# ChengeLi/LongTerm360FoV

Hardware: AMD Instinct MI355X
Metric: sequences/sec (batch=1024, T_in=30->T_out=30, h=256) (higher is better)
Workload: dtype f32; 1 GPU; configs[1]: target-only seq2seq inference (encoder + autoregressive decoder), H=256, batch=1024 per GPU, T_in=30->T_out=30, F_enc=90, F_dec=6, fp32, act=sigmoid, impl=auto; global_batch=1024, parallelism=replicas x1 (no collective)

## Files before the change

longterm360fov_amd/csrc/lstm_cluster.hip:

```cpp
#include <stdlib.h>

#include <atomic>
#include <mutex>

#include "fov_common.h"
#include "xch_common.h"

namespace fov {

constexpr int BT = 16;
constexpr int XR = 6;
constexpr int KPAD = 2;
constexpr int NXBUF = 3;
constexpr int CL_MAX_F = 96;
constexpr int CL_MAX_O = 8;
constexpr unsigned SPIN_LIMIT = 1u << 20;

constexpr int MODE_LAYER = 0;
constexpr int MODE_DECODE = 1;
constexpr int MODE_LAYER_ZX = 2;

typedef unsigned u32x2 __attribute__((ext_vector_type(2)));
typedef unsigned u32x4g __attribute__((ext_vector_type(4)));
typedef float f32x2 __attribute__((ext_vector_type(2)));
// ... 25 lines not shown
        if (stamp_on && t < STAMP_STEPS) {                                                      \
            unsigned long long t_;                                                              \
            asm volatile("s_memtime %0\n\ts_waitcnt lgkmcnt(0)" : "=s"(t_)::"memory");          \
            g_stamps[MODE & 1][t][slot] = t_;                                                       \
        }                                                                                       \
        __builtin_amdgcn_sched_barrier(0);                                                      \
    } while (0)
#define FOV_PSTAMP(slot)                                                                        \
    do {                                                                                        \
        __builtin_amdgcn_sched_barrier(0);                                                      \
        if (blockIdx.x == 5 && threadIdx.x == 0) g_stamps[MODE & 1][STAMP_STEPS - 1][slot] = __builtin_amdgcn_s_memtime(); \
        __builtin_amdgcn_sched_barrier(0);                                                      \
    } while (0)
#else
#define FOV_STAMP(slot) do { } while (0)
#define FOV_PSTAMP(slot) do { } while (0)
#endif

struct ClusterLds {
    int ldx, ldh;
    int off_k, off_h, off_x, off_w, off_bd, off_flag, total_floats;
};
__host__ __device__ inline ClusterLds cluster_lds(int H, int F, bool decode) {
    ClusterLds L;
    const int fp = round16(F);
    L.ldx = fp + 4;
    L.ldh = H + 4;
    L.off_k = 0;
    L.off_h = L.off_k + fp * 256 + 4 * KPAD * 256;
    L.off_x = L.off_h + BT * L.ldh;
    L.off_w = L.off_x + NXBUF * BT * L.ldx;
    L.off_bd = L.off_w + (decode ? 2 * 4 * 128 : 0);
    L.off_flag = L.off_bd + 8;
    L.total_floats = L.off_flag + 8 + 64;
    return L;
}

constexpr int MF_MID = 0, MF_FIRST = 1, MF_LAST = 2;
#define FOV_MFMA_STR(pre, post) pre "v_mfma_f32_16x16x4_f32 %0, %1, %2, %0" post
template <bool W_AGPR>
__device__ __forceinline__ void mfma_f32(f32x4& acc, float a, float w, int pos) {
    if constexpr (W_AGPR) {
        if (pos == MF_MID) asm volatile(FOV_MFMA_STR("", "") : "+v"(acc) : "v"(a), "a"(w));
        else if (pos == MF_FIRST) asm volatile(FOV_MFMA_STR("s_nop 1\n\t", "") : "+v"(acc) : "v"(a), "a"(w));
        else if (pos == MF_LAST) asm volatile(FOV_MFMA_STR("", "\n\ts_nop 7\n\ts_nop 3") : "+v"(acc) : "v"(a), "a"(w));
        else asm volatile(FOV_MFMA_STR("s_nop 1\n\t", "\n\ts_nop 7\n\ts_nop 3") : "+v"(acc) : "v"(a), "a"(w));
    } else {
        if (pos == MF_MID) asm volatile(FOV_MFMA_STR("", "") : "+v"(acc) : "v"(a), "v"(w));
        else if (pos == MF_FIRST) asm volatile(FOV_MFMA_STR("s_nop 1\n\t", "") : "+v"(acc) : "v"(a), "v"(w));
        else if (pos == MF_LAST) asm volatile(FOV_MFMA_STR("", "\n\ts_nop 7\n\ts_nop 3") : "+v"(acc) : "v"(a), "v"(w));
        else asm volatile(FOV_MFMA_STR("s_nop 1\n\t", "\n\ts_nop 7\n\ts_nop 3") : "+v"(acc) : "v"(a), "v"(w));
    }
}
__host__ __device__ constexpr int mf_pos(bool first_run, bool last_run, bool is_first, bool is_last) {
    return ((first_run && is_first) ? MF_FIRST : 0) | ((last_run && is_last) ? MF_LAST : 0);
}

template <int H, bool DEC_KMAP, int J0, int J1, bool REST>
__device__ __forceinline__ void load_weights(float (&wR)[H / 16][4][4], float (&bias)[4], float* sKw,
                                             const float* K, const float* R, const float* b, int F, int Fp,
                                             int col0, int slice, int lane) {
    constexpr int G = H / 64;
    const int n = lane & 15, g4 = lane >> 4;
    const int H4 = 4 * H;
    {
        const __amdgpu_buffer_rsrc_t rrs = __builtin_amdgcn_make_buffer_rsrc(const_cast<float*>(R), 0, H * H4 * 4, 0x00020000);
        const unsigned voff = (unsigned)((4 * g4 * H4 + col0 + n) * 4);
#pragma unroll
        for (int j = J0; j < J1; ++j) {
            const unsigned kb = (unsigned)((((slice + (j >> 2)) & (G - 1)) * 64 + (j & 3) * 16) * H4 * 4);
#pragma unroll
            for (int s = 0; s < 4; ++s)
#pragma unroll
                for (int g = 0; g < 4; ++g)
                    wR[j][s][g] = __uint_as_float(__builtin_amdgcn_raw_buffer_load_b32(rrs, voff, kb + (unsigned)((s * H4 + g * H) * 4), 0));
        }
    }
    if constexpr (!REST) return;
    {
        const __amdgpu_buffer_rsrc_t brs = __builtin_amdgcn_make_buffer_rsrc(const_cast<float*>(b), 0, b ? H4 * 4 : 0, 0x00020000);
#pragma unroll
        for (int g = 0; g < 4; ++g) bias[g] = __uint_as_float(__builtin_amdgcn_raw_buffer_load_b32(brs, (unsigned)((g * H + col0 + n) * 4), 0, 0));
    }
    const int nq = Fp >> 4;
    constexpr int QMAX = CL_MAX_F / 16;
    const __amdgpu_buffer_rsrc_t krs = __builtin_amdgcn_make_buffer_rsrc(const_cast<float*>(K), 0, F * H4 * 4, 0x00020000);
    f32x4 kv[DEC_KMAP ? 1 : QMAX][4];
#pragma unroll
    for (int q = 0; q < (DEC_KMAP ? 1 : QMAX); ++q)
#pragma unroll
        for (int s = 0; s < 4; ++s) {
            const int k = DEC_KMAP ? (s < 2 ? 4 * s + g4 : F) : 16 * q + 4 * g4 + s;
            const unsigned voff = (unsigned)((k * H4 + col0 + n) * 4);
#pragma unroll
            for (int g = 0; g < 4; ++g)
                kv[q][s][g] = __uint_as_float(__builtin_amdgcn_raw_buffer_load_b32(krs, voff + (unsigned)(g * H * 4), 0, 0));
        }
#pragma unroll
    for (int q = 0; q < (DEC_KMAP ? 1 : QMAX); ++q)
        if (q < nq) {
#pragma unroll
            for (int s = 0; s < 4; ++s) *(f32x4*)(sKw + ((q * 4 + s) * 64 + lane) * 4) = kv[q][s];
        }
}

template <int H>
__device__ __forceinline__ void load_r_block(float (&wR)[H / 16][4][4], int j, const float* R, int col0, int slice, int lane) {
    constexpr int G = H / 64;
    const int n = lane & 15, g4 = lane >> 4;
    const int H4 = 4 * H;
    const __amdgpu_buffer_rsrc_t rrs = __builtin_amdgcn_make_buffer_rsrc(const_cast<float*>(R), 0, H * H4 * 4, 0x00020000);
    const unsigned voff = (unsigned)((4 * g4 * H4 + col0 + n) * 4);
    const unsigned kb = (unsigned)((((slice + (j >> 2)) & (G - 1)) * 64 + (j & 3) * 16) * H4 * 4);
#pragma unroll
    for (int s = 0; s < 4; ++s)
#pragma unroll
        for (int g = 0; g < 4; ++g)
            wR[j][s][g] = __uint_as_float(__builtin_amdgcn_raw_buffer_load_b32(rrs, voff, kb + (unsigned)((s * H4 + g * H) * 4), 0));
}
template <int H>
__device__ __forceinline__ void load_dec_small(float (&bias)[4], f32x4 (&kb)[2], const float* K, const float* b, int F, int col0, int lane) {
    const int n = lane & 15, g4 = lane >> 4;
    const int H4 = 4 * H;
    const __amdgpu_buffer_rsrc_t brs = __builtin_amdgcn_make_buffer_rsrc(const_cast<float*>(b), 0, b ? H4 * 4 : 0, 0x00020000);
#pragma unroll
    for (int g = 0; g < 4; ++g) bias[g] = __uint_as_float(__builtin_amdgcn_raw_buffer_load_b32(brs, (unsigned)((g * H + col0 + n) * 4), 0, 0));
    const __amdgpu_buffer_rsrc_t krs = __builtin_amdgcn_make_buffer_rsrc(const_cast<float*>(K), 0, F * H4 * 4, 0x00020000);
#pragma unroll
    for (int s = 0; s < 2; ++s) {
        const unsigned voff = (unsigned)(((4 * s + g4) * H4 + col0 + n) * 4);
#pragma unroll
        for (int g = 0; g < 4; ++g) kb[s][g] = __uint_as_float(__builtin_amdgcn_raw_buffer_load_b32(krs, voff + (unsigned)(g * H * 4), 0, 0));
    }
}

template <bool FIRST, bool LAST>
__device__ __forceinline__ void input_proj(f32x4 (&acc)[4], const float* arow, const float* sKw, int nq, int lane) {
    if (nq <= 0) return;
    const float* bl = sKw + lane * 4;
    f32x4 a = *(const f32x4*)arow;
    f32x4 b0 = *(const f32x4*)bl;
    f32x4 b1 = *(const f32x4*)(bl + 256);
    if (FIRST) asm volatile("s_nop 1" : "+v"(acc[0]), "+v"(acc[1]), "+v"(acc[2]), "+v"(acc[3]));
    for (int q = 0; q < nq - 1; ++q) {
        const f32x4 an = *(const f32x4*)(arow + 16 * (q + 1));
        const float* bq = bl + q * 1024;
#pragma unroll
        for (int s = 0; s < 4; ++s) {
            const f32x4 bn = *(const f32x4*)(bq + (s + 2) * 256);
#pragma unroll
            for (int g = 0; g < 4; ++g) mfma_f32<false>(acc[g], a[s], b0[g], MF_MID);
            b0 = b1;
            b1 = bn;
        }
        a = an;
    }
    const float* bq = bl + (nq - 1) * 1024;
#pragma unroll
    for (int s = 0; s < 4; ++s) {
        const f32x4 bn = *(const f32x4*)(bq + (s + 2) * 256);
#pragma unroll
        for (int g = 0; g < 4; ++g) mfma_f32<false>(acc[g], a[s], b0[g], mf_pos(false, LAST, false, s == 3 && g == 3));
        b0 = b1;
        b1 = bn;
    }
}

template <int NQC, bool FIRST, bool LAST>
__device__ __forceinline__ void input_proj_fixed(f32x4 (&acc)[4], const float* arow, const float* sKw, int lane) {
    const float* bl = sKw + lane * 4;
    f32x4 a = *(const f32x4*)arow;
    f32x4 b0 = *(const f32x4*)bl;
    f32x4 b1 = *(const f32x4*)(bl + 256);
#pragma unroll
    for (int q = 0; q < NQC; ++q) {
        f32x4 an = a;
        if (q + 1 < NQC) an = *(const f32x4*)(arow + 16 * (q + 1));
#pragma unroll
        for (int s = 0; s < 4; ++s) {
            f32x4 bn = b1;
            if (4 * q + s + 2 < 4 * NQC) bn = *(const f32x4*)(bl + (4 * q + s + 2) * 256);
#pragma unroll
            for (int g = 0; g < 4; ++g)
                mfma_f32<false>(acc[g], a[s], b0[g], mf_pos(FIRST, LAST, q == 0 && s == 0, q == NQC - 1 && s == 3 && g == 3));
            b0 = b1;
            b1 = bn;
        }
        a = an;
    }
}
template <bool FIRST, bool LAST>
__device__ __forceinline__ void input_proj_any(f32x4 (&acc)[4], const float* arow, const float* sKw, int nq, int lane) {
    if (nq == 6) input_proj_fixed<6, FIRST, LAST>(acc, arow, sKw, lane);
    else input_proj<FIRST, LAST>(acc, arow, sKw, nq, lane);
}

template <bool LAST>
__device__ __forceinline__ void input_proj_reg(f32x4 (&acc)[4], f32x4 y4, const f32x4 (&kb)[2]) {
#pragma unroll
    for (int s = 0; s < 2; ++s)
#pragma unroll
        for (int g = 0; g < 4; ++g) mfma_f32<false>(acc[g], y4[s], kb[s][g], mf_pos(true, LAST, s == 0, s == 1 && g == 3));
}

template <int H, int J0, int J1, bool FIRST, bool LAST>
__device__ __forceinline__ void recurrent(f32x4 (&acc)[4], const float* hrow, const float (&wR)[H / 16][4][4]) {
    if (J0 >= J1) return;
    f32x4 a = *(const f32x4*)(hrow + 16 * J0);
#pragma unroll
    for (int j = J0; j < J1; ++j) {
        f32x4 an = a;
        if (j + 1 < J1) an = *(const f32x4*)(hrow + 16 * (j + 1));
#pragma unroll
        for (int s = 0; s < 4; ++s)
#pragma unroll
            for (int g = 0; g < 4; ++g)
                mfma_f32<true>(acc[g], a[s], wR[j][s][g], mf_pos(FIRST, LAST, j == J0 && s == 0, j == J1 - 1 && s == 3 && g == 3));
        a = an;
    }
}

struct ClusterCarry {
    unsigned epoch;
    XchTicket ticket;
    bool same_xcd, aborted, xch_used;
    float c[4], h[4];
};

template <int H, int ACT, int MODE, int FUSED>
__device__ __forceinline__ void cluster_body(const LstmParams& p, ClusterCarry& cy) {
    constexpr int G = H / 64;
    constexpr int NQ = H / 16;
    constexpr int NG = (G - 1) * 2;
    constexpr bool LAYER = (MODE != MODE_DECODE);
    constexpr bool ZX = (MODE == MODE_LAYER_ZX);
    constexpr bool F1 = (FUSED == 1), F2 = (FUSED == 2);
    extern __shared__ __attribute__((aligned(16))) float smem[];

    const int tid = threadIdx.x, lane = tid & 63, wave = tid >> 6;
    const int n = lane & 15, g4 = lane >> 4;
    constexpr unsigned OORB = 0x80000000u;
#ifdef FOV_STAMPS
    if (blockIdx.x == 5 && tid == 0) g_stamps[MODE & 1][STAMP_STEPS - 1][0] = __builtin_amdgcn_s_memtime();
#endif
    float hcarry[BT * H / 256];
    if constexpr (F2) {
        const ClusterLds L1 = cluster_lds(H, p.F, false);
#pragma unroll
        for (int q = 0; q < BT * H / 256; ++q) {
            const int i = tid + 256 * q;
            hcarry[q] = smem[L1.off_h + (i / H) * L1.ldh + (i - (i / H) * H)];
        }
        __syncthreads();
    }
    int group, slice;
    if (G > 1 && ((p.num_groups & 7) == 0 || p.xcd_pad)) {
        group = (blockIdx.x / (8 * G)) * 8 + (blockIdx.x & 7);
        slice = (blockIdx.x >> 3) & (G - 1);
    } else {
        group = blockIdx.x / G;
        slice = blockIdx.x - group * G;
    }
    const int col0 = slice * 64 + wave * 16;

    const float* Kp = LAYER ? p.K : p.dK;
    const float* Rp = LAYER ? p.R : p.dR;
    const float* bp = LAYER ? p.b : p.db;
    const int F = LAYER ? (ZX ? 0 : p.F) : p.F_dec;
    const int steps = LAYER ? p.T : p.T_out;
    const int Fp = round16(F);
    const int nq = Fp >> 4;

    const ClusterLds L = cluster_lds(H, F, !LAYER);
    const int LDX = L.ldx, LDH = L.ldh;
    float* sK = smem + L.off_k;
    float* sH = smem + L.off_h;
    float* sX = smem + L.off_x;
    float* sY = smem + L.off_w;
    int* sFlag = (int*)(smem + L.off_flag);
    float* sKw = sK + wave * (nq * 4 + KPAD) * 256;

    const bool xch_used = (G > 1) && (!LAYER || p.T > 1 || F1);
    unsigned* sXch = (unsigned*)(sFlag + 4);
    const bool hdr = xch_used && !F2;
    unsigned hdr_base = 0, hdr_launch = 0;
    if (hdr && tid == 0) {
        hdr_base = xch_status_load(p.status + ST_EPOCH);
        hdr_launch = xch_status_load(p.status + ST_LAUNCHES);
    }
    float wR[NQ][4][4];
    float bias[4];
    constexpr int JA = NQ < 3 ? NQ : 3;
    constexpr int STREAM_LA = 3;
    f32x4 kb[2];
    if constexpr (F2) {
        load_dec_small<H>(bias, kb, Kp, bp, F, col0, lane);
    } else {
        load_weights<H, !LAYER, 0, JA, false>(wR, bias, sKw, Kp, Rp, bp, F, Fp, col0, slice, lane);
    }
    unsigned long long* hello = p.xch + (size_t)p.num_groups * 2 * BT * H + (size_t)group * G;
    const unsigned my_xcc = xcc_id();
    if (hdr && tid == 0) {
        sXch[0] = hdr_base;
        sXch[1] = hdr_launch;
        st_granule(hello + slice, (((unsigned long long)hdr_base + 1ull) << 32) | my_xcc);
        xch_count_arrival(p.status);
    }
    FOV_PSTAMP(3);
    if constexpr (!F2) load_weights<H, !LAYER, JA, NQ, true>(wR, bias, sKw, Kp, Rp, bp, F, Fp, col0, slice, lane);
    FOV_PSTAMP(2);
    const bool poisoned = hdr && xch_poisoned(p.status);
    const unsigned arrival = 0;
    if (tid == 0) { sFlag[0] = (poisoned || (F2 && cy.aborted)) ? 1 : 0; sFlag[1] = 0; }
    if (hdr && !poisoned && tid < G) {
        const unsigned long long hello_tag = (unsigned long long)sXch[0] + 1ull;
        unsigned long long hv = 0;
        unsigned spins = 0;
        while (true) {
            hv = ld_granule(hello + tid);
            if ((hv >> 32) == hello_tag) break;
            if (++spins > SPIN_LIMIT || ((spins & 63u) == 0 && xch_poisoned(p.status))) {
                xch_give_up(p.status);
                sFlag[0] = 1;
                break;
            }
            __builtin_amdgcn_s_sleep(4);
        }
        if ((unsigned)hv != my_xcc) sFlag[1] = 1;
    }
    FOV_PSTAMP(4);
    float xpre[2][XR];
    {
        const int xrw0 = tid >> 4, xcl0 = tid & 15;
        const bool xuse0 = LAYER && !ZX;
        const int b00 = group * BT;
        const int live0 = (group < p.num_tiles) ? (p.B - b00 < BT ? p.B - b00 : BT) : 0;
        const __amdgpu_buffer_rsrc_t xg0 = __builtin_amdgcn_make_buffer_rsrc(
            const_cast<float*>(xuse0 && live0 > 0 ? p.x + (size_t)b00 * p.T * F : nullptr), 0, xuse0 ? live0 * p.T * F * 4 : 0, 0x00020000);
#pragma unroll
        for (int tt = 0; tt < 2; ++tt)
#pragma unroll
            for (int i = 0; i < XR; ++i)
                xpre[tt][i] = __uint_as_float(__builtin_amdgcn_raw_buffer_load_b32(
                    xg0, (tt < steps && xcl0 + 16 * i < F) ? (unsigned)((xrw0 * p.T * F + xcl0 + 16 * i) * 4) : OORB, (unsigned)(tt * F * 4), 0));
    }
    for (int i = tid; i < NXBUF * BT * LDX; i += 256) sX[i] = 0.f;

    float wd[4];
    float bd4[4];
    if (!LAYER) {
        const int O = p.F_dec;
        const __amdgpu_buffer_rsrc_t wdrs = __builtin_amdgcn_make_buffer_rsrc(const_cast<float*>(p.dW), 0, H * O * 4, 0x00020000);
        const __amdgpu_buffer_rsrc_t bdrs = __builtin_amdgcn_make_buffer_rsrc(const_cast<float*>(p.dbias), 0, O * 4, 0x00020000);
#pragma unroll
        for (int ss = 0; ss < 4; ++ss) {
            const int unit = col0 + 4 * g4 + ss;
            const int o = 4 * (n & 3) + (n >> 2);
            wd[ss] = __uint_as_float(__builtin_amdgcn_raw_buffer_load_b32(wdrs, (o < O) ? (unsigned)((unit * O + o) * 4) : OORB, 0, 0));
        }
#pragma unroll
        for (int ss = 0; ss < 4; ++ss)
            bd4[ss] = __uint_as_float(__builtin_amdgcn_raw_buffer_load_b32(bdrs, (4 * ss + g4 < O) ? (unsigned)((4 * ss + g4) * 4) : OORB, 0, 0));
    }
    if constexpr (F2) {
#pragma unroll
        for (int j = 0; j < STREAM_LA; ++j) load_r_block<H>(wR, j, Rp, col0, slice, lane);
    } else if (!LAYER) {
        __syncthreads();
        kb[0] = *(const f32x4*)(sKw + lane * 4);
        kb[1] = *(const f32x4*)(sKw + 256 + lane * 4);
    }

    __syncthreads();
    FOV_PSTAMP(5);
    XchTicket ticket = {0u, 0u, 0u};
    if (xch_used && !F2) ticket = xch_ticket(sXch, arrival);
    if constexpr (F2) ticket = cy.ticket;
    unsigned epoch = F2 ? cy.epoch : ticket.base;
    const bool same_xcd = F2 ? cy.same_xcd : (xch_used && (sFlag[1] == 0) && (p.force_safe_exchange == 0));
    bool aborted = F2 ? cy.aborted : (xch_used && sFlag[0] != 0);
    if (xch_used && !F2 && tid == 0 && !same_xcd && !aborted)
        xch_count_safe(p.status, ticket);
#ifdef FOV_STAMPS
    const bool stamp_on = (blockIdx.x == 5 && tid == 0);
#endif
    const float* hrow = sH + n * LDH + 4 * g4;

    const __amdgpu_buffer_rsrc_t xrs = __builtin_amdgcn_make_buffer_rsrc(
        p.xch + (size_t)group * 2 * BT * H, 0, 2 * BT * H * (int)sizeof(unsigned long long), 0x00020000);
    const unsigned pub_off = (unsigned)((2 * g4) * H + col0 + n) * 16u;
    unsigned goff[NG > 0 ? NG : 1];
    int loff[NG > 0 ? NG : 1];
#pragma unroll
    for (int j = 0; j < NG; ++j) {
        const int idx = j * 256 + tid;
        const int rot = (idx >> 9) + 1, within = idx & 511;
        const int osl = (slice + rot) & (G - 1);
        goff[j] = (unsigned)((within >> 6) * H + osl * 64 + (within & 63)) * 16u;
        loff[j] = 2 * (within >> 6) * LDH + rot * 64 + (within & 63);
    }

    constexpr int NYG = (LAYER || G == 1) ? 0 : G;
    const __amdgpu_buffer_rsrc_t yrs = __builtin_amdgcn_make_buffer_rsrc(
        p.xch + (size_t)p.num_groups * 2 * BT * H + (size_t)p.num_groups * G + (size_t)group * 2 * G * 128, 0,
        LAYER ? 0 : 2 * G * 128 * (int)sizeof(unsigned long long), 0x00020000);
    const unsigned ypub_off = (unsigned)((slice * 64 + lane) * 16);
    const unsigned ygoff = (unsigned)(lane * 16);
    constexpr unsigned YPAR_BYTES = G * 64 * 16;
    constexpr int YPAR_LDS = 4 * 128;
    auto own_partial = [&](int par) -> f32x2 {
        const float* yb = sY + par * YPAR_LDS + lane * 2;
        const f32x2 a0 = *(const f32x2*)yb, a1 = *(const f32x2*)(yb + 128), a2 = *(const f32x2*)(yb + 256), a3 = *(const f32x2*)(yb + 384);
        return (a0 + a1) + (a2 + a3);
    };

    const bool h_zero = !F2 && p.h0 == nullptr;
    for (int tile = group; tile < p.num_tiles && !aborted; tile += p.num_groups) {
        const int b0 = tile * BT;
        const int live_rows = p.B - b0 < BT ? p.B - b0 : BT;
        const __amdgpu_buffer_rsrc_t c0rs = __builtin_amdgcn_make_buffer_rsrc(
            const_cast<float*>(p.c0 ? p.c0 + (size_t)b0 * H : nullptr), 0, p.c0 ? live_rows * H * 4 : 0, 0x00020000);
        const __amdgpu_buffer_rsrc_t h0rs = __builtin_amdgcn_make_buffer_rsrc(
            const_cast<float*>(p.h0 ? p.h0 + (size_t)b0 * H : nullptr), 0, p.h0 ? live_rows * H * 4 : 0, 0x00020000);
        float c[4], hcur[4];
#pragma unroll
        for (int r = 0; r < 4; ++r) {
            const unsigned off = (unsigned)(((4 * g4 + r) * H + col0 + n) * 4);
            if constexpr (F2) {
                c[r] = cy.c[r];
                hcur[r] = cy.h[r];
            } else {
                c[r] = __uint_as_float(__builtin_amdgcn_raw_buffer_load_b32(c0rs, off, 0, 0));
                hcur[r] = __uint_as_float(__builtin_amdgcn_raw_buffer_load_b32(h0rs, off, 0, 0));
            }
        }
        {
            float hv[BT * H / 256];
#pragma unroll
            for (int q = 0; q < BT * H / 256; ++q) {
                const int i = tid + 256 * q;
                const int row = i / H, pos = i - row * H;
                const int unit = ((slice + (pos >> 6)) & (G - 1)) * 64 + (pos & 63);
                if constexpr (F2) hv[q] = hcarry[q];
                else hv[q] = h_zero ? 0.f : __uint_as_float(__builtin_amdgcn_raw_buffer_load_b32(h0rs, (unsigned)((row * H + unit) * 4), 0, 0));
            }
#pragma unroll
            for (int q = 0; q < BT * H / 256; ++q) {
                const int i = tid + 256 * q;
                const int row = i / H, pos = i - row * H;
                sH[row * LDH + pos] = hv[q];
            }
        }
        const int xrw = tid >> 4, xcl = tid & 15;
        const bool xuse = LAYER && !ZX;
        const __amdgpu_buffer_rsrc_t xgrs = __builtin_amdgcn_make_buffer_rsrc(
            const_cast<float*>(xuse ? p.x + (size_t)b0 * p.T * F : nullptr), 0, xuse ? live_rows * p.T * F * 4 : 0, 0x00020000);
        unsigned xoff[XR];
#pragma unroll
        for (int i = 0; i < XR; ++i) xoff[i] = (xcl + 16 * i < F) ? (unsigned)((xrw * p.T * F + xcl + 16 * i) * 4) : OORB;
        const __amdgpu_buffer_rsrc_t zxrs = __builtin_amdgcn_make_buffer_rsrc(
            const_cast<float*>(ZX ? p.zx + (size_t)b0 * p.T * 4 * H : nullptr), 0, ZX ? live_rows * p.T * 4 * H * 4 : 0, 0x00020000);
        const unsigned zxoff = (unsigned)((4 * g4 * p.T * 4 * H + col0 + n) * 4);
        f32x4 zr[4];
        float* xl = sX + xrw * LDX + xcl;
        if (xuse) {
            float x2[2][XR];
            if (tile == group) {
#pragma unroll
                for (int tt = 0; tt < 2; ++tt)
#pragma unroll
                    for (int i = 0; i < XR; ++i) x2[tt][i] = xpre[tt][i];
            } else {
#pragma unroll
                for (int tt = 0; tt < 2; ++tt)
#pragma unroll
                    for (int i = 0; i < XR; ++i)
                        x2[tt][i] = __uint_as_float(__builtin_amdgcn_raw_buffer_load_b32(xgrs, tt < steps ? xoff[i] : OORB, (unsigned)(tt * F * 4), 0));
            }
#pragma unroll
            for (int tt = 0; tt < 2; ++tt)
                if (tt < steps) {
#pragma unroll
                    for (int i = 0; i < XR; ++i)
                        if (xcl + 16 * i < F) xl[tt * BT * LDX + 16 * i] = x2[tt][i];
                }
        }
        const __amdgpu_buffer_rsrc_t yors = __builtin_amdgcn_make_buffer_rsrc(
            (!LAYER && p.out) ? p.out + (size_t)b0 * p.T_out * p.F_dec : nullptr, 0, (!LAYER && p.out) ? live_rows * p.T_out * p.F_dec * 4 : 0, 0x00020000);
        unsigned yoff[2];
#pragma unroll
        for (int ss = 0; ss < 2; ++ss)
            yoff[ss] = (!LAYER && 4 * ss + g4 < p.F_dec) ? (unsigned)((n * p.T_out * p.F_dec + 4 * ss + g4) * 4) : OORB;
        f32x4 y4 = (f32x4){0.f, 0.f, 0.f, 0.f};
        if (!LAYER) {
            const __amdgpu_buffer_rsrc_t y0rs = __builtin_amdgcn_make_buffer_rsrc(
                const_cast<float*>(p.dec_in0 + (size_t)b0 * F), 0, live_rows * F * 4, 0x00020000);
#pragma unroll
            for (int ss = 0; ss < 4; ++ss)
                y4[ss] = __uint_as_float(__builtin_amdgcn_raw_buffer_load_b32(y0rs, (4 * ss + g4 < F) ? (unsigned)((n * F + 4 * ss + g4) * 4) : OORB, 0, 0));
        }
        __syncthreads();
        FOV_PSTAMP(6);

        f32x4 acc[4];
#pragma unroll
        for (int g = 0; g < 4; ++g) acc[g] = (f32x4){bias[g], bias[g], bias[g], bias[g]};
        if (ZX && steps > 0) {
#pragma unroll
            for (int g = 0; g < 4; ++g)
#pragma unroll
                for (int r = 0; r < 4; ++r)
                    acc[g][r] = bias[g] + __uint_as_float(__builtin_amdgcn_raw_buffer_load_b32(zxrs, zxoff + (unsigned)((r * p.T * 4 * H + g * H) * 4), 0, 0));
        }
        if (steps > 0) {
            if (LAYER) input_proj_any<true, true>(acc, sX + n * LDX + 4 * g4, sKw, nq, lane);
            else input_proj_reg<true>(acc, y4, kb);
            if constexpr (F2) {
                f32x4 a = *(const f32x4*)hrow;
#pragma unroll
                for (int j = 0; j < NQ; ++j) {
                    if (j + STREAM_LA < NQ) load_r_block<H>(wR, j + STREAM_LA, Rp, col0, slice, lane);
                    f32x4 an = a;
                    if (j + 1 < NQ) an = *(const f32x4*)(hrow + 16 * (j + 1));
#pragma unroll
                    for (int s2 = 0; s2 < 4; ++s2)
#pragma unroll
                        for (int g = 0; g < 4; ++g)
                            mfma_f32<true>(acc[g], a[s2], wR[j][s2][g], mf_pos(false, true, false, j == NQ - 1 && s2 == 3 && g == 3));
                    a = an;
                }
            } else if (!h_zero) {
                recurrent<H, 0, 4, true, true>(acc, hrow, wR);
            }
        }

        float xr[XR];
#pragma unroll
        for (int i = 0; i < XR; ++i) xr[i] = 0.f;
        for (int t = 0; t < steps; ++t) {
            FOV_STAMP(0);
#ifdef FOV_STAMPS
            if (stamp_on && t < STAMP_STEPS) g_stamps[MODE & 1][t][9] = __builtin_amdgcn_s_memrealtime();
#endif
            if (LAYER && !ZX && t > 0 && t + 1 < steps) {
                float* xb = xl + ((t + 1) % 3) * BT * LDX;
#pragma unroll
                for (int i = 0; i < XR; ++i)
                    if (xcl + 16 * i < F) xb[16 * i] = xr[i];
            }
            if (ZX && t + 1 < steps) {
#pragma unroll
                for (int g = 0; g < 4; ++g)
#pragma unroll
                    for (int r = 0; r < 4; ++r)
                        zr[g][r] = bias[g] + __uint_as_float(__builtin_amdgcn_raw_buffer_load_b32(
                                                 zxrs, zxoff + (unsigned)(((r * p.T + (t + 1)) * 4 * H + g * H) * 4), 0, 0));
            }
            if (LAYER && !ZX && t + 2 < steps) {
#pragma unroll
                for (int i = 0; i < XR; ++i)
                    xr[i] = __uint_as_float(__builtin_amdgcn_raw_buffer_load_b32(xgrs, xoff[i], (unsigned)((t + 2) * F * 4), 0));
            }
            if (LAYER || t == 0) {
                if (!((h_zero || F2) && t == 0)) recurrent<H, 4, NQ, true, true>(acc, hrow, wR);
            } else {
                constexpr int JM = 4 + (NQ - 4) / 2;
                recurrent<H, 4, JM, true, false>(acc, hrow, wR);
                u32x4g vy[NYG > 0 ? NYG : 1];
                const unsigned yso = (epoch & 1u) * YPAR_BYTES;
#pragma unroll
                for (int q = 0; q < NYG; ++q) vy[q] = __builtin_amdgcn_raw_buffer_load_b128(yrs, ygoff, yso + (unsigned)(q * 1024), 16);
                recurrent<H, JM, NQ, false, false>(acc, hrow, wR);
                __builtin_amdgcn_sched_barrier(0);
                f32x2 ysum;
                if constexpr (NYG > 0) {
                    unsigned spins = 0;
                    while (true) {
                        bool ok = true;
#pragma unroll
                        for (int q = 0; q < NYG; ++q) ok = ok && (vy[q].y == epoch) && (vy[q].w == epoch);
                        if (__all(ok)) break;
                        if (++spins > SPIN_LIMIT || ((spins & 63u) == 0 && xch_poisoned(p.status))) {
                            if (lane == 0) { xch_give_up(p.status); sFlag[0] = 1; }
// ... 32 lines not shown
                const float ig = acc[0][r], fg = acc[1][r], gg = acc[2][r], og = acc[3][r];
                c[r] = fmaf(fg, c[r], ig * gg);
                hcur[r] = og * c[r];
#else
                const float ig = rec_act<ACT>(acc[0][r]);
                const float fg = rec_act<ACT>(acc[1][r]);
                const float gg = tanh_f(acc[2][r]);
                const float og = rec_act<ACT>(acc[3][r]);
                c[r] = fmaf(fg, c[r], ig * gg);
                hcur[r] = og * tanh_f(c[r]);
#endif
                if (LAYER && p.reserve) {
                    const int row = b0 + 4 * g4 + r;
                    if (row < p.B) {
                        float* rp = p.reserve + (((size_t)row * p.T + t) * 5) * H + col0 + n;
                        rp[0] = ig; rp[H] = fg; rp[2 * H] = gg; rp[3 * H] = og; rp[4 * H] = c[r];
                    }
                }
            }
            unsigned xsoff = 0;
            const bool do_xch = (G > 1) && (!LAYER || t + 1 < steps || F1);
            if (do_xch) {
                ++epoch;
                xsoff = (epoch & 1u) * (unsigned)(BT * H * sizeof(unsigned long long));
                if (same_xcd) {
#pragma unroll
                    for (int r = 0; r < 2; ++r)
                        __builtin_amdgcn_raw_buffer_store_b128((u32x4g){__float_as_uint(hcur[2 * r]), epoch, __float_as_uint(hcur[2 * r + 1]), epoch},
                                                               xrs, pub_off + r * H * 16, xsoff, 1 );
                } else {
#pragma unroll
                    for (int r = 0; r < 2; ++r)
                        __builtin_amdgcn_raw_buffer_store_b128((u32x4g){__float_as_uint(hcur[2 * r]), epoch, __float_as_uint(hcur[2 * r + 1]), epoch},
                                                               xrs, pub_off + r * H * 16, xsoff, 16 );
                }
            }
            if (LAYER && p.hs) {
#pragma unroll
                for (int r = 0; r < 4; ++r) {
                    const int row = b0 + 4 * g4 + r;
                    if (row < p.B) p.hs[((size_t)row * p.T + t) * H + col0 + n] = hcur[r];
                }
            }
            FOV_STAMP(2);
            FOV_STAMP(3);
#pragma unroll
            for (int r = 0; r < 4; ++r) sH[(4 * g4 + r) * LDH + wave * 16 + n] = hcur[r];
            __syncthreads();
            FOV_STAMP(4);
            const bool more = (t + 1 < steps);
            if (more) {
#pragma unroll
                for (int g = 0; g < 4; ++g) acc[g] = ZX ? zr[g] : (f32x4){bias[g], bias[g], bias[g], bias[g]};
                if (LAYER) input_proj_any<true, false>(acc, sX + ((t + 1) % 3) * BT * LDX + n * LDX + 4 * g4, sKw, nq, lane);
            }
            FOV_STAMP(5);
            u32x4g v[NG > 0 ? NG : 1];
            constexpr int GJ = LAYER ? 0 : 1;
            if (more) {
                recurrent<H, 0, GJ, true, false>(acc, hrow, wR);
                if (do_xch) {
#pragma unroll
                    for (int j = 0; j < NG; ++j) v[j] = __builtin_amdgcn_raw_buffer_load_b128(xrs, goff[j], xsoff, 16);
                }
                recurrent<H, GJ, 4, LAYER, (G == 1)>(acc, hrow, wR);
            } else if (do_xch) {
#pragma unroll
                for (int j = 0; j < NG; ++j) v[j] = __builtin_amdgcn_raw_buffer_load_b128(xrs, goff[j], xsoff, 16);
            }
            FOV_STAMP(11);
            if (!LAYER) {
                const f32x4 hb = *(const f32x4*)(hrow + 16 * wave);
                f32x4 dacc[2];
                dacc[0] = (f32x4){0.f, 0.f, 0.f, 0.f};
                dacc[1] = (f32x4){0.f, 0.f, 0.f, 0.f};
#ifndef FOV_DBG_NODENSE
#pragma unroll
                for (int ss = 0; ss < 4; ++ss)
                    mfma_f32<false>(dacc[ss & 1], wd[ss], hb[ss], mf_pos(true, true, ss < 2, ss == 3));
#endif
                *(f32x2*)(sY + (t & 1) * YPAR_LDS + wave * 128 + lane * 2) = (f32x2){dacc[0][0] + dacc[1][0], dacc[0][1] + dacc[1][1]};
            }
            if (do_xch) {
                unsigned spins = 0;
#ifdef FOV_DBG_NOGATHER
                while (false) {
#else
                while (true) {
#endif
                    bool ok = true;
#pragma unroll
                    for (int j = 0; j < NG; ++j) ok = ok && (v[j].y == epoch) && (v[j].w == epoch);
                    if (__all(ok)) break;
                    ++spins;
                    if (spins > SPIN_LIMIT || ((spins & 63u) == 0 && xch_poisoned(p.status))) {
                        if (lane == 0) {
                            xch_give_up(p.status);
                            sFlag[0] = 1;
                        }
                        break;
                    }
                    __builtin_amdgcn_s_sleep(1);
                    asm volatile("" ::: "memory");
#pragma unroll
                    for (int j = 0; j < NG; ++j) v[j] = __builtin_amdgcn_raw_buffer_load_b128(xrs, goff[j], xsoff, 16);
                }
#ifdef FOV_STAMPS
// ... 49 lines not shown
                        for (int q = 0; q < w2; ++q) P[q] += P[q + w2];
                    ysum = P[0];
                } else {
                    ysum = own_partial((steps - 1) & 1);
                }
                if (got) {
#pragma unroll
                    for (int ss = 0; ss < 2; ++ss)
                        __builtin_amdgcn_raw_buffer_store_b32(__float_as_uint(tanh_f(ysum[ss] + bd4[ss])), yors, yoff[ss],
                                                              (unsigned)((steps - 1) * p.F_dec * 4), 0);
                }
            }
        }
        if constexpr (F1) {
#pragma unroll
            for (int r = 0; r < 4; ++r) { cy.c[r] = c[r]; cy.h[r] = hcur[r]; }
        }
        if (!aborted && !F1) {
#pragma unroll
            for (int r = 0; r < 4; ++r) {
                const int row = b0 + 4 * g4 + r;
                if (row < p.B) {
                    if (p.hT) p.hT[(size_t)row * H + col0 + n] = hcur[r];
                    if (p.cT) p.cT[(size_t)row * H + col0 + n] = c[r];
                }
            }
        }
#ifdef FOV_STAMPS
        if (blockIdx.x == 5 && tid == 0) g_stamps[MODE & 1][STAMP_STEPS - 1][1] = __builtin_amdgcn_s_memtime();
#endif
        if constexpr (FUSED != 0) break;
    }
    if constexpr (F1) {
        cy.epoch = epoch; cy.ticket = ticket; cy.same_xcd = same_xcd; cy.aborted = aborted; cy.xch_used = xch_used;
        __syncthreads();
    } else {
        if (xch_used) xch_settle(p.status, ticket, (unsigned)p.epoch_span);
    }
}

template <int H, int ACT, int MODE>
__global__ __launch_bounds__(256, 1) void lstm_cluster_kernel(LstmParams p) {
    if constexpr (H >= 128) {
        if (p.xcd_pad && (int)((blockIdx.x / (8 * (H / 64))) * 8 + (blockIdx.x & 7)) >= p.num_groups) {
            const bool exchanging = (MODE == MODE_DECODE) || p.T > 1;
            if (threadIdx.x == 0 && exchanging) xch_count_arrival(p.status);
            return;
        }
    }
    ClusterCarry cy;
    cluster_body<H, ACT, MODE, 0>(p, cy);
}

template <int H, int ACT>
__global__ __launch_bounds__(256, 1) void lstm_cluster_fused_kernel(LstmParams p) {
    if constexpr (H >= 128) {
        if (p.xcd_pad && (int)((blockIdx.x / (8 * (H / 64))) * 8 + (blockIdx.x & 7)) >= p.num_groups) {
            if (threadIdx.x == 0) xch_count_arrival(p.status);
            return;
        }
    }
    ClusterCarry cy;
    cluster_body<H, ACT, MODE_LAYER, 1>(p, cy);
    cluster_body<H, ACT, MODE_DECODE, 2>(p, cy);
}

int device_cu_count() {
    static std::atomic<int> cus[64];
    int dev = 0;
    if (hipGetDevice(&dev) != hipSuccess || dev < 0 || dev >= 64) return 256;
    int n = cus[dev].load(std::memory_order_relaxed);
    if (n == 0) {
        hipDeviceProp_t prop;
        n = (hipGetDeviceProperties(&prop, dev) == hipSuccess && prop.multiProcessorCount > 0) ? prop.multiProcessorCount : 256;
        cus[dev].store(n, std::memory_order_relaxed);
    }
    const int lim = env_knobs().resident_limit;
    return (lim > 0 && lim < n) ? lim : n;
}

int ensure_dynamic_lds(const void* kern, size_t lds, int block) {
    struct Seen { const void* k; size_t lds; int dev; };
    static Seen seen[256];
    static int n_seen = 0;
    static std::mutex mu;
    int dev = 0;
    (void)hipGetDevice(&dev);
    std::lock_guard<std::mutex> lock(mu);
    for (int i = 0; i < n_seen; ++i)
        if (seen[i].k == kern && seen[i].dev == dev && seen[i].lds >= lds) return FOV_OK;
    hipError_t e = hipFuncSetAttribute(kern, hipFuncAttributeMaxDynamicSharedMemorySize, (int)lds);
    if (e != hipSuccess) { set_error("hipFuncSetAttribute: %s", hipGetErrorString(e)); return FOV_ERR_LAUNCH; }
    int per_cu = 0;
    e = hipOccupancyMaxActiveBlocksPerMultiprocessor(&per_cu, kern, block, lds);
    if (e != hipSuccess || per_cu < 1) {
        (void)hipGetLastError();
        set_error("persistent kernel: a %d-thread workgroup with %zu B of LDS is not resident on this device (occupancy %d)", block, lds, per_cu);
        return FOV_ERR_UNSUPPORTED;
    }
    if (n_seen < 256) seen[n_seen++] = Seen{kern, lds, dev};
    return FOV_OK;
}

bool cluster_shape_ok(int F, int H) {
    return (H == 64 || H == 128 || H == 256) && F >= 1 && F <= CL_MAX_F;
}

int cluster_num_groups(int B, int H) {
    const int G = H / 64;
    const int tiles = (B + BT - 1) / BT;
    const int groups = device_cu_count() / G;
    if (groups < 1) return 0;
    return tiles < groups ? (tiles > 0 ? tiles : 1) : groups;
}

static size_t cluster_xch_bytes(int B, int H) {
    const size_t groups = (size_t)cluster_num_groups(B, H);
    const size_t b = (groups * 2 * BT * H + groups * (H / 64) + groups * 2 * (H / 64) * 128) * sizeof(unsigned long long);
    return (b + 255) & ~(size_t)255;
}

size_t cluster_workspace_bytes(int B, int H) {
    (void)cluster_xch_bytes;
    return kStatusBytes + kXchBytes + (size_t)2 * B * H * sizeof(float);
}

template <int H>
static int launch_cluster_h(const LstmParams& p, int mode, hipStream_t stream) {
    void (*kern)(LstmParams) = nullptr;
    if (mode == MODE_LAYER && p.zx) mode = MODE_LAYER_ZX;
    if (p.act == FOV_ACT_HARD_SIGMOID)
        kern = mode == MODE_DECODE ? lstm_cluster_kernel<H, FOV_ACT_HARD_SIGMOID, MODE_DECODE>
               : mode == MODE_LAYER_ZX ? lstm_cluster_kernel<H, FOV_ACT_HARD_SIGMOID, MODE_LAYER_ZX>
                                       : lstm_cluster_kernel<H, FOV_ACT_HARD_SIGMOID, MODE_LAYER>;
    else
        kern = mode == MODE_DECODE ? lstm_cluster_kernel<H, FOV_ACT_SIGMOID, MODE_DECODE>
               : mode == MODE_LAYER_ZX ? lstm_cluster_kernel<H, FOV_ACT_SIGMOID, MODE_LAYER_ZX>
                                       : lstm_cluster_kernel<H, FOV_ACT_SIGMOID, MODE_LAYER>;
    const int F = mode == MODE_DECODE ? p.F_dec : (p.zx ? 0 : p.F);
    const ClusterLds L = cluster_lds(H, F, mode == MODE_DECODE);
    const size_t lds = (size_t)L.total_floats * sizeof(float);
    if (lds > 160 * 1024) {
        set_error("cluster kernel: H=%d F=%d needs %zu B of LDS (> 160 KiB)", H, F, lds);
        return FOV_ERR_UNSUPPORTED;
    }
    int rc = ensure_dynamic_lds((const void*)kern, lds);
    if (rc) return rc;
    LstmParams q = p;
    const int padded = xch_padded_groups(q.num_groups);
    q.xcd_pad = (H >= 128 && !env_knobs().no_xcd_pad && (q.num_groups & 7) != 0 && device_cu_count() >= padded * (H / 64)) ? 1 : 0;
    const dim3 grid((q.xcd_pad ? padded : q.num_groups) * (H / 64)), block(256);
    hipLaunchKernelGGL(kern, grid, block, lds, stream, q);
    return launch_check("cluster");
}

template <int H>
static int launch_cluster_fused_h(const LstmParams& p, hipStream_t stream) {
    void (*kern)(LstmParams) = p.act == FOV_ACT_HARD_SIGMOID ? lstm_cluster_fused_kernel<H, FOV_ACT_HARD_SIGMOID>
                                                             : lstm_cluster_fused_kernel<H, FOV_ACT_SIGMOID>;
    const ClusterLds L1 = cluster_lds(H, p.F, false), L2 = cluster_lds(H, p.F_dec, true);
    const size_t lds = (size_t)(L1.total_floats > L2.total_floats ? L1.total_floats : L2.total_floats) * sizeof(float);
    if (lds > 160 * 1024) { set_error("fused cluster kernel: needs %zu B of LDS (> 160 KiB)", lds); return FOV_ERR_UNSUPPORTED; }
    int rc = ensure_dynamic_lds((const void*)kern, lds);
    if (rc) return rc;
    LstmParams q = p;
    const bool no_pad = env_knobs().no_xcd_pad != 0;
    const int padded = (q.num_groups + 7) & ~7;
    q.xcd_pad = (H >= 128 && !no_pad && (q.num_groups & 7) != 0 && device_cu_count() >= padded * (H / 64)) ? 1 : 0;
    hipLaunchKernelGGL(kern, dim3((q.xcd_pad ? padded : q.num_groups) * (H / 64)), dim3(256), lds, stream, q);
    return launch_check("fused cluster");
}

static int launch_cluster_fused(const LstmParams& p, hipStream_t stream) {
    switch (p.H) {
        case 64: return launch_cluster_fused_h<64>(p, stream);
        case 128: return launch_cluster_fused_h<128>(p, stream);
        default: return launch_cluster_fused_h<256>(p, stream);
    }
}

static int launch_cluster_mode(const LstmParams& p, int mode, hipStream_t stream) {
    switch (p.H) {
        case 64: return launch_cluster_h<64>(p, mode, stream);
        case 128: return launch_cluster_h<128>(p, mode, stream);
        default: return launch_cluster_h<256>(p, mode, stream);
    }
}

int launch_cluster(const LstmParams& p_in, bool decode, hipStream_t stream) {
    LstmParams p = p_in;
    if (p.B == 0) return FOV_OK;
    if (p.zx) p.F = 1;
    if (!cluster_shape_ok(p.F, p.H) || (decode && (p.F_dec < 1 || p.F_dec > CL_MAX_O))) {
        set_error("cluster kernel supports H in {64,128,256}, 1<=F<=%d, F_dec<=%d (got H=%d F=%d F_dec=%d)",
                  CL_MAX_F, CL_MAX_O, p.H, p.F, p.F_dec);
        return FOV_ERR_UNSUPPORTED;
    }
    p.num_tiles = (p.B + BT - 1) / BT;
    p.num_groups = cluster_num_groups(p.B, p.H);
    if (p.num_groups < 1) { set_error("cluster kernel: fewer than %d CUs available for one group", p.H / 64); return FOV_ERR_UNSUPPORTED; }
    p.force_safe_exchange = env_knobs().force_safe_exchange;
    if (cluster_xch_bytes(p.B, p.H) > kXchBytes - kHelloBytes) { set_error("cluster kernel: granule area exceeds the workspace's"); return FOV_ERR_WORKSPACE; }
    const int visits = (p.num_tiles + p.num_groups - 1) / p.num_groups;
    if (!decode) {
        p.epoch_span = p.T * visits + 1;
        if (int rc_ = xch_account(p.status, p.epoch_span, stream)) return rc_;
        return launch_cluster_mode(p, MODE_LAYER, stream);
    }

    if (visits == 1 && p.T > 0 && p.T_out > 0 && !p.hs && !p.reserve && !env_knobs().two_launches) {
        LstmParams f = p;
        f.epoch_span = p.T + p.T_out + 2;
// ... 43 lines not shown
```

Baseline: 3.017 million sequences/s.

## Overlap recurrent weight streaming with prologue handshake and first input projection

Restructures the fused kernel prologue so the K and bias loads are issued early and written to LDS later, and the XCD hello handshake's first load and status word are issued before the recurrent weight blocks load. In the fused encoder, recurrent weight blocks are streamed in stages: some before the first barrier, the rest interleaved with the first-step input projection through a per-k-block hook, with a specialized fixed six-block path chosen when the padded feature count is 96. It also skips loading h0 when it is zero and adds empty asm clobbers to close MFMA accumulator chains. The aim is to hide the global weight-load latency of the startup phase behind other work, at the cost of higher register pressure and an extra template instantiation.

```diff
diff --git a/longterm360fov_amd/csrc/lstm_cluster.hip b/longterm360fov_amd/csrc/lstm_cluster.hip
--- a/longterm360fov_amd/csrc/lstm_cluster.hip
+++ b/longterm360fov_amd/csrc/lstm_cluster.hip
@@ -101,42 +101,25 @@
         else asm volatile(FOV_MFMA_STR("s_nop 1\n\t", "\n\ts_nop 7\n\ts_nop 3") : "+v"(acc) : "v"(a), "v"(w));
     }
 }
+__device__ __forceinline__ void mfma_close(f32x4 (&acc)[4]) {
+    asm volatile("" : "+v"(acc[0]), "+v"(acc[1]), "+v"(acc[2]), "+v"(acc[3]));
+}
 __host__ __device__ constexpr int mf_pos(bool first_run, bool last_run, bool is_first, bool is_last) {
     return ((first_run && is_first) ? MF_FIRST : 0) | ((last_run && is_last) ? MF_LAST : 0);
 }
 
-template <int H, bool DEC_KMAP, int J0, int J1, bool REST>
-__device__ __forceinline__ void load_weights(float (&wR)[H / 16][4][4], float (&bias)[4], float* sKw,
-                                             const float* K, const float* R, const float* b, int F, int Fp,
-                                             int col0, int slice, int lane) {
-    constexpr int G = H / 64;
+template <int H, bool DEC_KMAP, int KQ>
+__device__ __forceinline__ void request_k_bias(f32x4 (&kv)[KQ][4], float (&bias)[4], const float* K, const float* b, int F,
+                                               int col0, int lane) {
+    static_assert(KQ == (DEC_KMAP ? 1 : CL_MAX_F / 16), "one k-block for the decoder, the widest input otherwise");
     const int n = lane & 15, g4 = lane >> 4;
     const int H4 = 4 * H;
-    {
-        const __amdgpu_buffer_rsrc_t rrs = __builtin_amdgcn_make_buffer_rsrc(const_cast<float*>(R), 0, H * H4 * 4, 0x00020000);
-        const unsigned voff = (unsigned)((4 * g4 * H4 + col0 + n) * 4);
-#pragma unroll
-        for (int j = J0; j < J1; ++j) {
-            const unsigned kb = (unsigned)((((slice + (j >> 2)) & (G - 1)) * 64 + (j & 3) * 16) * H4 * 4);
-#pragma unroll
-            for (int s = 0; s < 4; ++s)
-#pragma unroll
-                for (int g = 0; g < 4; ++g)
-                    wR[j][s][g] = __uint_as_float(__builtin_amdgcn_raw_buffer_load_b32(rrs, voff, kb + (unsigned)((s * H4 + g * H) * 4), 0));
-        }
-    }
-    if constexpr (!REST) return;
-    {
-        const __amdgpu_buffer_rsrc_t brs = __builtin_amdgcn_make_buffer_rsrc(const_cast<float*>(b), 0, b ? H4 * 4 : 0, 0x00020000);
-#pragma unroll
-        for (int g = 0; g < 4; ++g) bias[g] = __uint_as_float(__builtin_amdgcn_raw_buffer_load_b32(brs, (unsigned)((g * H + col0 + n) * 4), 0, 0));
-    }
-    const int nq = Fp >> 4;
-    constexpr int QMAX = CL_MAX_F / 16;
+    const __amdgpu_buffer_rsrc_t brs = __builtin_amdgcn_make_buffer_rsrc(const_cast<float*>(b), 0, b ? H4 * 4 : 0, 0x00020000);
+#pragma unroll
+    for (int g = 0; g < 4; ++g) bias[g] = __uint_as_float(__builtin_amdgcn_raw_buffer_load_b32(brs, (unsigned)((g * H + col0 + n) * 4), 0, 0));
     const __amdgpu_buffer_rsrc_t krs = __builtin_amdgcn_make_buffer_rsrc(const_cast<float*>(K), 0, F * H4 * 4, 0x00020000);
-    f32x4 kv[DEC_KMAP ? 1 : QMAX][4];
-#pragma unroll
-    for (int q = 0; q < (DEC_KMAP ? 1 : QMAX); ++q)
+#pragma unroll
+    for (int q = 0; q < KQ; ++q)
 #pragma unroll
         for (int s = 0; s < 4; ++s) {
             const int k = DEC_KMAP ? (s < 2 ? 4 * s + g4 : F) : 16 * q + 4 * g4 + s;
@@ -145,8 +128,11 @@
             for (int g = 0; g < 4; ++g)
                 kv[q][s][g] = __uint_as_float(__builtin_amdgcn_raw_buffer_load_b32(krs, voff + (unsigned)(g * H * 4), 0, 0));
         }
-#pragma unroll
-    for (int q = 0; q < (DEC_KMAP ? 1 : QMAX); ++q)
+}
+template <int KQ>
+__device__ __forceinline__ void commit_k(const f32x4 (&kv)[KQ][4], float* sKw, int nq, int lane) {
+#pragma unroll
+    for (int q = 0; q < KQ; ++q)
         if (q < nq) {
 #pragma unroll
             for (int s = 0; s < 4; ++s) *(f32x4*)(sKw + ((q * 4 + s) * 64 + lane) * 4) = kv[q][s];
@@ -165,7 +151,7 @@
     for (int s = 0; s < 4; ++s)
 #pragma unroll
         for (int g = 0; g < 4; ++g)
-            wR[j][s][g] = __uint_as_float(__builtin_amdgcn_raw_buffer_load_b32(rrs, voff, kb + (unsigned)((s * H4 + g * H) * 4), 0));
+            wR[j][s][g] = __uint_as_float(__builtin_amdgcn_raw_buffer_load_b32(rrs, voff + (unsigned)(g * H * 4), kb + (unsigned)(s * H4 * 4), 0));
 }
 template <int H>
 __device__ __forceinline__ void load_dec_small(float (&bias)[4], f32x4 (&kb)[2], const float* K, const float* b, int F, int col0, int lane) {
@@ -213,16 +199,21 @@
         b0 = b1;
         b1 = bn;
     }
-}
-
-template <int NQC, bool FIRST, bool LAST>
-__device__ __forceinline__ void input_proj_fixed(f32x4 (&acc)[4], const float* arow, const float* sKw, int lane) {
+    if (LAST) mfma_close(acc);
+}
+
+struct NoHook {
+    __device__ __forceinline__ void operator()(int) const {}
+};
+template <int NQC, bool FIRST, bool LAST, class Hook = NoHook>
+__device__ __forceinline__ void input_proj_fixed(f32x4 (&acc)[4], const float* arow, const float* sKw, int lane, const Hook& hook = Hook()) {
     const float* bl = sKw + lane * 4;
     f32x4 a = *(const f32x4*)arow;
     f32x4 b0 = *(const f32x4*)bl;
     f32x4 b1 = *(const f32x4*)(bl + 256);
 #pragma unroll
     for (int q = 0; q < NQC; ++q) {
+        hook(q);
         f32x4 an = a;
         if (q + 1 < NQC) an = *(const f32x4*)(arow + 16 * (q + 1));
 #pragma unroll
@@ -237,6 +228,7 @@
         }
         a = an;
     }
+    if (LAST) mfma_close(acc);
 }
 template <bool FIRST, bool LAST>
 __device__ __forceinline__ void input_proj_any(f32x4 (&acc)[4], const float* arow, const float* sKw, int nq, int lane) {
@@ -250,6 +242,7 @@
     for (int s = 0; s < 2; ++s)
 #pragma unroll
         for (int g = 0; g < 4; ++g) mfma_f32<false>(acc[g], y4[s], kb[s][g], mf_pos(true, LAST, s == 0, s == 1 && g == 3));
+    if (LAST) mfma_close(acc);
 }
 
 template <int H, int J0, int J1, bool FIRST, bool LAST>
@@ -267,6 +260,7 @@
                 mfma_f32<true>(acc[g], a[s], wR[j][s][g], mf_pos(FIRST, LAST, j == J0 && s == 0, j == J1 - 1 && s == 3 && g == 3));
         a = an;
     }
+    if (LAST) mfma_close(acc);
 }
 
 struct ClusterCarry {
@@ -276,7 +270,7 @@
     float c[4], h[4];
 };
 
-template <int H, int ACT, int MODE, int FUSED>
+template <int H, int ACT, int MODE, int FUSED, bool X6 = false>
 __device__ __forceinline__ void cluster_body(const LstmParams& p, ClusterCarry& cy) {
     constexpr int G = H / 64;
     constexpr int NQ = H / 16;
@@ -339,45 +333,14 @@
     }
     float wR[NQ][4][4];
     float bias[4];
-    constexpr int JA = NQ < 3 ? NQ : 3;
     constexpr int STREAM_LA = 3;
+    constexpr int JA = NQ < STREAM_LA ? NQ : STREAM_LA;
+    constexpr int JB = NQ < 6 ? NQ : 6;
     f32x4 kb[2];
-    if constexpr (F2) {
-        load_dec_small<H>(bias, kb, Kp, bp, F, col0, lane);
-    } else {
-        load_weights<H, !LAYER, 0, JA, false>(wR, bias, sKw, Kp, Rp, bp, F, Fp, col0, slice, lane);
-    }
-    unsigned long long* hello = p.xch + (size_t)p.num_groups * 2 * BT * H + (size_t)group * G;
-    const unsigned my_xcc = xcc_id();
-    if (hdr && tid == 0) {
-        sXch[0] = hdr_base;
-        sXch[1] = hdr_launch;
-        st_granule(hello + slice, (((unsigned long long)hdr_base + 1ull) << 32) | my_xcc);
-        xch_count_arrival(p.status);
-    }
-    FOV_PSTAMP(3);
-    if constexpr (!F2) load_weights<H, !LAYER, JA, NQ, true>(wR, bias, sKw, Kp, Rp, bp, F, Fp, col0, slice, lane);
-    FOV_PSTAMP(2);
-    const bool poisoned = hdr && xch_poisoned(p.status);
-    const unsigned arrival = 0;
-    if (tid == 0) { sFlag[0] = (poisoned || (F2 && cy.aborted)) ? 1 : 0; sFlag[1] = 0; }
-    if (hdr && !poisoned && tid < G) {
-        const unsigned long long hello_tag = (unsigned long long)sXch[0] + 1ull;
-        unsigned long long hv = 0;
-        unsigned spins = 0;
-        while (true) {
-            hv = ld_granule(hello + tid);
-            if ((hv >> 32) == hello_tag) break;
-            if (++spins > SPIN_LIMIT || ((spins & 63u) == 0 && xch_poisoned(p.status))) {
-                xch_give_up(p.status);
-                sFlag[0] = 1;
-                break;
-            }
-            __builtin_amdgcn_s_sleep(4);
-        }
-        if ((unsigned)hv != my_xcc) sFlag[1] = 1;
-    }
-    FOV_PSTAMP(4);
+    constexpr int KQ = LAYER ? CL_MAX_F / 16 : 1;
+    f32x4 kv[KQ][4];
+    if constexpr (F2) load_dec_small<H>(bias, kb, Kp, bp, F, col0, lane);
+    else request_k_bias<H, !LAYER, KQ>(kv, bias, Kp, bp, F, col0, lane);
     float xpre[2][XR];
     {
         const int xrw0 = tid >> 4, xcl0 = tid & 15;
@@ -393,8 +356,6 @@
                 xpre[tt][i] = __uint_as_float(__builtin_amdgcn_raw_buffer_load_b32(
                     xg0, (tt < steps && xcl0 + 16 * i < F) ? (unsigned)((xrw0 * p.T * F + xcl0 + 16 * i) * 4) : OORB, (unsigned)(tt * F * 4), 0));
     }
-    for (int i = tid; i < NXBUF * BT * LDX; i += 256) sX[i] = 0.f;
-
     float wd[4];
     float bd4[4];
     if (!LAYER) {
@@ -411,11 +372,48 @@
         for (int ss = 0; ss < 4; ++ss)
             bd4[ss] = __uint_as_float(__builtin_amdgcn_raw_buffer_load_b32(bdrs, (4 * ss + g4 < O) ? (unsigned)((4 * ss + g4) * 4) : OORB, 0, 0));
     }
-    if constexpr (F2) {
-#pragma unroll
-        for (int j = 0; j < STREAM_LA; ++j) load_r_block<H>(wR, j, Rp, col0, slice, lane);
-    } else if (!LAYER) {
-        __syncthreads();
+    unsigned long long* hello = p.xch + (size_t)p.num_groups * 2 * BT * H + (size_t)group * G;
+    const unsigned my_xcc = xcc_id();
+    if (hdr && tid == 0) {
+        sXch[0] = hdr_base;
+        sXch[1] = hdr_launch;
+        st_granule(hello + slice, (((unsigned long long)hdr_base + 1ull) << 32) | my_xcc);
+        xch_count_arrival(p.status);
+    }
+    FOV_PSTAMP(3);
+    const __amdgpu_buffer_rsrc_t strs = __builtin_amdgcn_make_buffer_rsrc(p.status, 0, hdr ? 256 : 0, 0x00020000);
+    const unsigned pword = __builtin_amdgcn_raw_buffer_load_b32(strs, hdr ? (unsigned)(ST_TIMEOUT * 4) : OORB, 0, 16 );
+    for (int i = tid; i < NXBUF * BT * LDX; i += 256) sX[i] = 0.f;
+    if constexpr (!F2) commit_k<KQ>(kv, sKw, nq, lane);
+    FOV_PSTAMP(2);
+    const __amdgpu_buffer_rsrc_t hers = __builtin_amdgcn_make_buffer_rsrc(hello, 0, hdr ? G * 8 : 0, 0x00020000);
+    const u32x2 hv0 = __builtin_amdgcn_raw_buffer_load_b64(hers, (hdr && tid < G) ? (unsigned)(tid * 8) : OORB, 0, 16 );
+#pragma unroll
+    for (int j = 0; j < JA; ++j) load_r_block<H>(wR, j, Rp, col0, slice, lane);
+    if constexpr (FUSED == 0) {
+#pragma unroll
+        for (int j = JA; j < NQ; ++j) load_r_block<H>(wR, j, Rp, col0, slice, lane);
+    }
+    const bool poisoned = hdr && xch_timeout_set(pword);
+    const unsigned arrival = 0;
+    if (tid == 0) { sFlag[0] = (poisoned || (F2 && cy.aborted)) ? 1 : 0; sFlag[1] = 0; }
+    if (hdr && !poisoned && tid < G) {
+        const unsigned long long hello_tag = (unsigned long long)sXch[0] + 1ull;
+        unsigned long long hv = ((unsigned long long)hv0.y << 32) | hv0.x;
+        unsigned spins = 0;
+        while ((hv >> 32) != hello_tag) {
+            if (++spins > SPIN_LIMIT || ((spins & 63u) == 0 && xch_poisoned(p.status))) {
+                xch_give_up(p.status);
+                sFlag[0] = 1;
+                break;
+            }
+            __builtin_amdgcn_s_sleep(4);
+            hv = ld_granule(hello + tid);
+        }
+        if ((unsigned)hv != my_xcc) sFlag[1] = 1;
+    }
+    FOV_PSTAMP(4);
+    if (!F2 && !LAYER) {
         kb[0] = *(const f32x4*)(sKw + lane * 4);
         kb[1] = *(const f32x4*)(sKw + 256 + lane * 4);
     }
@@ -483,7 +481,7 @@
                 hcur[r] = __uint_as_float(__builtin_amdgcn_raw_buffer_load_b32(h0rs, off, 0, 0));
             }
         }
-        {
+        if (F2 || !h_zero) {
             float hv[BT * H / 256];
 #pragma unroll
             for (int q = 0; q < BT * H / 256; ++q) {
@@ -491,13 +489,20 @@
                 const int row = i / H, pos = i - row * H;
                 const int unit = ((slice + (pos >> 6)) & (G - 1)) * 64 + (pos & 63);
                 if constexpr (F2) hv[q] = hcarry[q];
-                else hv[q] = h_zero ? 0.f : __uint_as_float(__builtin_amdgcn_raw_buffer_load_b32(h0rs, (unsigned)((row * H + unit) * 4), 0, 0));
+                else hv[q] = __uint_as_float(__builtin_amdgcn_raw_buffer_load_b32(h0rs, (unsigned)((row * H + unit) * 4), 0, 0));
             }
 #pragma unroll
             for (int q = 0; q < BT * H / 256; ++q) {
                 const int i = tid + 256 * q;
                 const int row = i / H, pos = i - row * H;
                 sH[row * LDH + pos] = hv[q];
+            }
+        } else {
+#pragma unroll
+            for (int q = 0; q < BT * H / 256; ++q) {
+                const int i = tid + 256 * q;
+                const int row = i / H, pos = i - row * H;
+                sH[row * LDH + pos] = 0.f;
             }
         }
         const int xrw = tid >> 4, xcl = tid & 15;
@@ -548,6 +553,10 @@
             for (int ss = 0; ss < 4; ++ss)
                 y4[ss] = __uint_as_float(__builtin_amdgcn_raw_buffer_load_b32(y0rs, (4 * ss + g4 < F) ? (unsigned)((n * F + 4 * ss + g4) * 4) : OORB, 0, 0));
         }
+        if constexpr (F1) {
+#pragma unroll
+            for (int j = JA; j < JB; ++j) load_r_block<H>(wR, j, Rp, col0, slice, lane);
+        }
         __syncthreads();
         FOV_PSTAMP(6);
 
@@ -561,8 +570,21 @@
                 for (int r = 0; r < 4; ++r)
                     acc[g][r] = bias[g] + __uint_as_float(__builtin_amdgcn_raw_buffer_load_b32(zxrs, zxoff + (unsigned)((r * p.T * 4 * H + g * H) * 4), 0, 0));
         }
-        if (steps > 0) {
-            if (LAYER) input_proj_any<true, true>(acc, sX + n * LDX + 4 * g4, sKw, nq, lane);
+        if (F1 || steps > 0) {
+            if constexpr (F1) {
+                const float* arow = sX + n * LDX + 4 * g4;
+                if constexpr (X6) {
+                    input_proj_fixed<6, true, true>(acc, arow, sKw, lane, [&](int q) __attribute__((always_inline)) {
+                        if (JB + q < NQ) load_r_block<H>(wR, JB + q, Rp, col0, slice, lane);
+                    });
+#pragma unroll
+                    for (int j = JB + 6; j < NQ; ++j) load_r_block<H>(wR, j, Rp, col0, slice, lane);
+                } else {
+#pragma unroll
+                    for (int j = JB; j < NQ; ++j) load_r_block<H>(wR, j, Rp, col0, slice, lane);
+                    input_proj<true, true>(acc, arow, sKw, nq, lane);
+                }
+            } else if (LAYER) input_proj_any<true, true>(acc, sX + n * LDX + 4 * g4, sKw, nq, lane);
             else input_proj_reg<true>(acc, y4, kb);
             if constexpr (F2) {
                 f32x4 a = *(const f32x4*)hrow;
@@ -578,6 +600,7 @@
                             mfma_f32<true>(acc[g], a[s2], wR[j][s2][g], mf_pos(false, true, false, j == NQ - 1 && s2 == 3 && g == 3));
                     a = an;
                 }
+                mfma_close(acc);
             } else if (!h_zero) {
                 recurrent<H, 0, 4, true, true>(acc, hrow, wR);
             }
@@ -716,7 +739,9 @@
             if (more) {
 #pragma unroll
                 for (int g = 0; g < 4; ++g) acc[g] = ZX ? zr[g] : (f32x4){bias[g], bias[g], bias[g], bias[g]};
-                if (LAYER) input_proj_any<true, false>(acc, sX + ((t + 1) % 3) * BT * LDX + n * LDX + 4 * g4, sKw, nq, lane);
+                if constexpr (X6) input_proj_fixed<6, true, false>(acc, sX + ((t + 1) % 3) * BT * LDX + n * LDX + 4 * g4, sKw, lane);
+                else if constexpr (F1) input_proj<true, false>(acc, sX + ((t + 1) % 3) * BT * LDX + n * LDX + 4 * g4, sKw, nq, lane);
+                else if (LAYER) input_proj_any<true, false>(acc, sX + ((t + 1) % 3) * BT * LDX + n * LDX + 4 * g4, sKw, nq, lane);
             }
             FOV_STAMP(5);
             u32x4g v[NG > 0 ? NG : 1];
@@ -872,7 +897,7 @@
     cluster_body<H, ACT, MODE, 0>(p, cy);
 }
 
-template <int H, int ACT>
+template <int H, int ACT, bool X6>
 __global__ __launch_bounds__(256, 1) void lstm_cluster_fused_kernel(LstmParams p) {
     if constexpr (H >= 128) {
         if (p.xcd_pad && (int)((blockIdx.x / (8 * (H / 64))) * 8 + (blockIdx.x & 7)) >= p.num_groups) {
@@ -881,7 +906,7 @@
         }
     }
     ClusterCarry cy;
-    cluster_body<H, ACT, MODE_LAYER, 1>(p, cy);
+    cluster_body<H, ACT, MODE_LAYER, 1, X6>(p, cy);
     cluster_body<H, ACT, MODE_DECODE, 2>(p, cy);
 }
 
@@ -976,8 +1001,10 @@
 
 template <int H>
 static int launch_cluster_fused_h(const LstmParams& p, hipStream_t stream) {
-    void (*kern)(LstmParams) = p.act == FOV_ACT_HARD_SIGMOID ? lstm_cluster_fused_kernel<H, FOV_ACT_HARD_SIGMOID>
-                                                             : lstm_cluster_fused_kernel<H, FOV_ACT_SIGMOID>;
+    const bool x6 = round16(p.F) == 96;
+    void (*kern)(LstmParams) = p.act == FOV_ACT_HARD_SIGMOID
+                                   ? (x6 ? lstm_cluster_fused_kernel<H, FOV_ACT_HARD_SIGMOID, true> : lstm_cluster_fused_kernel<H, FOV_ACT_HARD_SIGMOID, false>)
+                                   : (x6 ? lstm_cluster_fused_kernel<H, FOV_ACT_SIGMOID, true> : lstm_cluster_fused_kernel<H, FOV_ACT_SIGMOID, false>);
     const ClusterLds L1 = cluster_lds(H, p.F, false), L2 = cluster_lds(H, p.F_dec, true);
     const size_t lds = (size_t)(L1.total_floats > L2.total_floats ? L1.total_floats : L2.total_floats) * sizeof(float);
     if (lds > 160 * 1024) { set_error("fused cluster kernel: needs %zu B of LDS (> 160 KiB)", lds); return FOV_ERR_UNSUPPORTED; }
```

New measurement: 3.048 million sequences/s, median of 3. Within noise of the previous version (+1.0%).
